# marsupialtail/quokka

Measured on AMD Instinct MI355X. Metric: rows/s, higher is better.
Workload: dtype f64; 1 GPU; TPC-H SF100 Q1, fused filter+group-by, 600037900 lineitem rows/GPU resident in HBM (BASELINE.json configs[1]); rows_per_gpu=600037900, query=Q1

## Files before the change

include/quokka_amd.h:

```cpp
#ifndef QUOKKA_AMD_H
#define QUOKKA_AMD_H

#include <stdint.h>

#ifdef __cplusplus
extern "C" {
#endif

int qk_init(int device);
int qk_device_count(int *out);
const char *qk_last_error(void);
const char *qk_build_arch(void);

int qk_dmalloc(uint64_t nbytes, void **dptr);
int qk_hmalloc_impl(uint64_t nbytes, void **hptr);
int qk_hfree(void *hptr);
int qk_dfree(void *dptr);
int qk_h2d(void *dst_dev, const void *src_host, uint64_t nbytes);
int qk_d2h(void *dst_host, const void *src_dev, uint64_t nbytes);
int qk_h2d_async(void *stream, void *dst_dev, const void *src_host,
                 uint64_t nbytes);
int qk_d2h_async(void *stream, void *dst_host, const void *src_dev,
                 uint64_t nbytes);
int qk_dmemset(void *dst_dev, int value, uint64_t nbytes);
int qk_fill_i64(void *stream, int64_t *dst_dev, int64_t value, uint64_t n);

int qk_stream_create(void **stream);
int qk_stream_destroy(void *stream);
int qk_stream_sync(void *stream);
int qk_event_create(void **ev);
int qk_event_destroy(void *ev);
int qk_event_record(void *ev, void *stream);
int qk_stream_wait_event(void *stream, void *ev);
int qk_timer_create(void **timer);
int qk_timer_destroy(void *timer);
int qk_timer_start(void *timer, void *stream);
int qk_timer_stop(void *timer, void *stream);
int qk_timer_elapsed_ms(void *timer, float *out_ms);

int qk_gen_lineitem(void *stream, uint64_t n, uint64_t row_offset, uint64_t seed,
                    int64_t n_parts, int64_t n_suppliers, int64_t n_orders,
                    int64_t *l_orderkey, int64_t *l_suppkey,
                    double *l_quantity, double *l_extendedprice,
                    double *l_discount, double *l_tax,
                    uint8_t *l_returnflag, uint8_t *l_linestatus,
                    int32_t *l_shipdate, int32_t *l_commitdate,
                    int32_t *l_receiptdate);

int qk_gen_orders(void *stream, uint64_t n, uint64_t row_offset, uint64_t seed,
                  int64_t n_customers, int64_t *o_orderkey, int64_t *o_custkey,
                  int32_t *o_orderdate, int32_t *o_shippriority,
                  uint8_t *o_orderpriority, double *o_totalprice,
                  int64_t li_n_parts);
int qk_gen_customer(void *stream, uint64_t n, uint64_t row_offset,
                    uint64_t seed, int64_t *c_custkey, uint8_t *c_mktsegment,
                    int32_t *c_nationkey);
int qk_gen_supplier(void *stream, uint64_t n, uint64_t row_offset,
                    uint64_t seed, int64_t *s_suppkey, int32_t *s_nationkey);
int qk_gen_aux(void *stream, uint64_t n, uint64_t row_offset, uint64_t seed,
               uint64_t salt, int mode, int64_t a, int64_t b,
               uint8_t *out_u8, double *out_f64);

int qk_q1_agg(void *stream, uint64_t n,
              const int32_t *l_shipdate, const double *l_quantity,
              const double *l_extendedprice, const double *l_discount,
              const double *l_tax, const uint8_t *l_returnflag,
              const uint8_t *l_linestatus, int32_t cutoff_date,
              double *out_dev );

int qk_q6_agg(void *stream, uint64_t n,
              const int32_t *l_shipdate, const double *l_quantity,
              const double *l_extendedprice, const double *l_discount,
              int32_t date_lo, int32_t date_hi,
              double disc_lo, double disc_hi, double qty_hi,
              double *out_dev );

int qk_filter_i32(void *stream, uint64_t n, const int32_t *col, int op,
                  int32_t value, uint32_t *out_idx, uint64_t *out_count_dev);
int qk_filter_u8(void *stream, uint64_t n, const uint8_t *col, int op,
                 uint8_t value, uint32_t *out_idx, uint64_t *out_count_dev);
int qk_filter_f64(void *stream, uint64_t n, const double *col, int op,
                  double value, uint32_t *out_idx, uint64_t *out_count_dev);

int qk_flag_gt_i32(void *stream, uint64_t n, const int32_t *a,
                   const int32_t *b, double *out);
int qk_mul_1md(void *stream, uint64_t n, const double *a, const double *b,
               double *out);

int qk_gather_i64(void *stream, uint64_t n_idx, const uint32_t *idx,
                  const int64_t *src, int64_t *dst);
int qk_gather_f64(void *stream, uint64_t n_idx, const uint32_t *idx,
                  const double *src, double *dst);
int qk_gather_i32(void *stream, uint64_t n_idx, const uint32_t *idx,
                  const int32_t *src, int32_t *dst);
int qk_gather_u8(void *stream, uint64_t n_idx, const uint32_t *idx,
                 const uint8_t *src, uint8_t *dst);

#define QK_JOIN_EMPTY INT64_MIN
int qk_join_build(void *stream, uint64_t n_build, const int64_t *keys,
                  uint32_t build_row_offset, int64_t *slot_keys,
                  int32_t *slot_head, int32_t *chain_next, uint64_t capacity);
int qk_join_probe(void *stream, uint64_t n_probe, const int64_t *keys,
                  const int64_t *slot_keys, const int32_t *slot_head,
                  const int32_t *chain_next, uint64_t capacity, int mode,
                  uint32_t *out_probe_idx, uint32_t *out_build_idx,
                  uint64_t out_capacity, uint64_t *out_cursor_dev);

int qk_build_u8eq(void *stream, uint64_t n, const int64_t *keys,
                  const uint8_t *flag, uint8_t flag_val, int64_t *slot_keys,
                  int32_t *slot_head, uint64_t capacity, uint32_t *bloom,
                  uint64_t bloom_mask);
int qk_q3_build_orders(void *stream, uint64_t n, const int64_t *o_orderkey,
                       const int64_t *o_custkey, const int32_t *o_orderdate,
                       int32_t date_lt, const int64_t *cust_keys,
                       const int32_t *cust_head, uint64_t cust_cap,
                       int64_t *slot_keys, int32_t *slot_head,
                       uint64_t capacity, uint32_t *bloom,
                       uint64_t bloom_mask, const uint32_t *cust_bloom,
                       uint64_t cust_bloom_mask);
int qk_q3_count_orders(void *stream, uint64_t n, const int64_t *o_custkey,
                       const int32_t *o_orderdate, int32_t date_lt,
                       const int64_t *cust_keys, const int32_t *cust_head,
                       uint64_t cust_cap, uint64_t *count_dev,
                       const uint32_t *cust_bloom, uint64_t cust_bloom_mask);
int qk_q3_probe_agg(void *stream, uint64_t n, const int64_t *l_orderkey,
                    const int32_t *l_shipdate, const double *l_price,
                    const double *l_disc, int32_t date_gt,
                    const int64_t *slot_keys, const int32_t *slot_head,
                    uint64_t capacity, double *slot_sums ,
                    uint64_t *match_count_dev );
int qk_q3_probe_agg_nt(void *stream, uint64_t n, const int64_t *l_orderkey,
                       const int32_t *l_shipdate, const double *l_price,
                       const double *l_disc, int32_t date_gt,
                       const int64_t *slot_keys, const int32_t *slot_head,
                       uint64_t capacity, double *slot_sums,
                       uint64_t *match_count_dev, const uint32_t *bloom,
                       uint64_t bloom_mask);
int qk_q3_probe_agg_nt4(void *stream, uint64_t n, const int64_t *l_orderkey,
                        const int32_t *l_shipdate, const double *l_price,
                        const double *l_disc, int32_t date_gt,
                        const int64_t *slot_keys, const int32_t *slot_head,
                        uint64_t capacity, double *slot_sums,
                        uint64_t *match_count_dev, const uint32_t *bloom,
                        uint64_t bloom_mask);
int qk_q3_extract(void *stream, const int64_t *slot_keys,
                  const int32_t *slot_head, const double *slot_sums,
                  uint64_t capacity, int64_t *out_keys, int32_t *out_row,
                  double *out_sums, uint64_t out_cap, uint64_t *cursor_dev);

int qk_build_keyval_i32(void *stream, uint64_t n, const int64_t *keys,
                        const int32_t *vals, uint32_t accept_mask,
                        int64_t *slot_keys, int32_t *slot_val,
                        uint64_t capacity, uint32_t *bloom,
                        uint64_t bloom_mask);
int qk_q5_build_orders(void *stream, uint64_t n, const int64_t *o_orderkey,
                       const int64_t *o_custkey, const int32_t *o_orderdate,
                       int32_t date_lo, int32_t date_hi,
                       const int64_t *cust_keys, const int32_t *cust_val,
                       uint64_t cust_cap, int64_t *slot_keys,
                       int32_t *slot_val, uint64_t capacity,
                       uint64_t *count_dev, uint32_t *bloom,
                       uint64_t bloom_mask, const uint32_t *cust_bloom,
                       uint64_t cust_bloom_mask);
int qk_q5_probe_agg(void *stream, uint64_t n, const int64_t *l_orderkey,
                    const int64_t *l_suppkey, const double *l_price,
                    const double *l_disc, const int64_t *ord_keys,
                    const int32_t *ord_val, uint64_t ord_cap,
                    const int64_t *supp_keys, const int32_t *supp_val,
                    uint64_t supp_cap, double *out25,
                    uint64_t *match_count_dev );

int qk_q5_probe_agg_nt(void *stream, uint64_t n, const int64_t *l_orderkey,
                       const int64_t *l_suppkey, const double *l_price,
                       const double *l_disc, const int64_t *ord_keys,
                       const int32_t *ord_val, uint64_t ord_cap,
                       const int64_t *supp_keys, const int32_t *supp_val,
                       uint64_t supp_cap, double *out25,
                       uint64_t *match_count_dev, const uint32_t *bloom,
                       uint64_t bloom_mask);

int qk_groupby_i64_sum(void *stream, uint64_t n, const int64_t *keys,
                       const void *vals_dev ,
                       const int32_t *agg_ops_dev ,
                       int nvals, int rstride ,
                       int64_t *table, uint64_t cap, uint64_t *n_inserted);
int qk_groupby_init(void *stream, int64_t *table, uint64_t cap, int rstride,
                    int nvals, const double *inits_dev);
int qk_fill_f64(void *stream, double *dst_dev, double value, uint64_t n);
int qk_groupby_extract(void *stream, const int64_t *table, int rstride,
                       int nvals, uint64_t cap, int64_t *out_keys,
                       double *out_sums ,
                       uint64_t out_cap, uint64_t *cursor);
int qk_groupby_extract_gt(void *stream, const int64_t *table, int rstride,
                          int nvals, uint64_t cap, int col, double threshold,
                          int64_t *out_keys, double *out_sums,
                          uint64_t out_cap, uint64_t *cursor);

int qk_partition_hist(void *stream, uint64_t n, const int64_t *keys,
                      uint32_t nparts, uint64_t *hist_dev);
int qk_partition_scatter(void *stream, uint64_t n, const int64_t *keys,
                         uint32_t nparts, uint64_t *cursors_dev,
                         uint32_t *out_idx);

int qk_sort_pairs_u64(void *stream, uint64_t n, uint64_t *keys,
                      uint32_t *payload, uint64_t *keys_tmp,
                      uint32_t *pay_tmp, int npasses);
int qk_map_f64_u64(void *stream, uint64_t n, const double *in, uint64_t *out);
int qk_map_i64_u64(void *stream, uint64_t n, const int64_t *in,
                   uint64_t *out);
int qk_iota_u32(void *stream, uint64_t n, uint32_t *out);
int qk_bnot_u64(void *stream, uint64_t n, uint64_t *x);

const char *qk_jit_last_error(void);
int qk_jit_filter_build(const char *c_expr, int ncols, const int *coltypes,
                        void **prog_out);
int qk_jit_filter_run(void *prog, void *stream, uint64_t n,
                      const void *const *col_ptrs, uint32_t *out_idx,
                      uint64_t *count_dev);
int qk_jit_map_build(const char *c_expr, int ncols, const int *coltypes,
                     void **prog_out);
int qk_jit_map_run(void *prog, void *stream, uint64_t n,
                   const void *const *col_ptrs, double *out_dev);
int qk_jit_agg_build(const char *pred_or_empty, const char *group_expr,
                     int ngroups, int naggs, const char *const *agg_exprs,
                     const int *agg_ops, int ncols, const int *coltypes,
                     void **prog_out);
int qk_jit_agg_run(void *prog, void *stream, uint64_t n,
                   const void *const *col_ptrs, double *out_dev);
int qk_jit_filter_free(void *prog);
uint64_t qk_jit_code_size(void *prog);

#define QK_UID_BYTES 128
int qk_comm_unique_id(uint8_t out[QK_UID_BYTES]);
int qk_comm_init(int rank, int world, const uint8_t uid[QK_UID_BYTES],
                 void **comm_out);
int qk_comm_destroy(void *comm);
int qk_alltoallv(void *stream, void *comm, int world, uint32_t elem_size,
                 const void *send_buf, const uint64_t *send_offsets,
                 const uint64_t *send_counts, void *recv_buf,
                 const uint64_t *recv_offsets, const uint64_t *recv_counts);
int qk_allreduce_f64(void *stream, void *comm, double *buf, uint64_t n);

int qk_pq_plain_copy(void *stream, uint64_t ntiles, const uint64_t *tiles,
                     const void *src_bytes, void *dst, uint32_t elem_size);
int qk_pq_rle_pages(void *stream, uint64_t npages, const uint64_t *ents,
                    const uint8_t *src_bytes, uint32_t *out);
int qk_str_dict_encode(void *stream, uint64_t n, const int64_t *offsets,
                       const uint8_t *bytes, uint64_t *slot_hash,
                       int32_t *slot_code, uint64_t capacity,
                       uint64_t *code_off, uint32_t *code_len,
                       uint8_t *arena, uint64_t *arena_cursor_dev,
                       uint32_t *counter_dev, uint32_t *out_codes);
int qk_str_dict_rehash(void *stream, uint32_t ncodes,
                       const uint64_t *code_off, const uint32_t *code_len,
                       const uint8_t *arena, uint64_t *slot_hash,
                       int32_t *slot_code, uint64_t capacity);
#define QK_LIKE_MAX_PAT 256
#define QK_LIKE_MAX_SEGS 16
typedef struct {
  uint32_t nseg;
  uint8_t anchor_start;
  uint8_t anchor_end;
  uint8_t exact;
  uint8_t pad_;
  uint16_t seg_off[QK_LIKE_MAX_SEGS];
  uint16_t seg_len[QK_LIKE_MAX_SEGS];
  uint32_t wild[QK_LIKE_MAX_PAT / 32];
  uint8_t pat[QK_LIKE_MAX_PAT];
} qk_like_pat;
int qk_like_compile(const uint8_t *pat, uint32_t len, int exact,
                    qk_like_pat *out);
int qk_str_like_i32(void *stream, uint64_t n, const int32_t *offsets,
                    const uint8_t *bytes, const qk_like_pat *pat, int negate,
                    uint8_t *out_flags);
int qk_str_like_i64(void *stream, uint64_t n, const int64_t *offsets,
                    const uint8_t *bytes, const qk_like_pat *pat, int negate,
                    uint8_t *out_flags);
int qk_str_like_path_i32(void *stream, uint64_t n, const int32_t *offsets,
                         const uint8_t *bytes, const qk_like_pat *pat,
                         int negate, int stage, uint8_t *out_flags);
int qk_str_like_path_i64(void *stream, uint64_t n, const int64_t *offsets,
                         const uint8_t *bytes, const qk_like_pat *pat,
                         int negate, int stage, uint8_t *out_flags);
int qk_str_like_host_i64(uint64_t n, const int64_t *offsets,
                         const uint8_t *bytes, const qk_like_pat *pat,
                         int negate, uint8_t *out_flags);
int qk_like_tile_bytes(void);
int qk_i64_combine(void *stream, uint64_t n, const int64_t *x,
                   const int64_t *y, int64_t scale, int64_t *out);
int qk_i64_shr(void *stream, uint64_t n, const int64_t *x, int shift,
               int64_t *out);
int qk_d2d(void *dst_dev, const void *src_dev, uint64_t nbytes);

int qk_snappy_pages(void *stream, uint64_t npages, const uint64_t *descs_dev,
                    const uint8_t *src_dev, uint8_t *dst_dev,
                    int64_t *out_dev);
int qk_gzip_pages(void *stream, uint64_t npages, const uint64_t *descs_dev,
                  const uint8_t *src_dev, uint8_t *dst_dev,
                  int64_t *out_dev);
#define QK_PQ_PAGE_FIELDS 10
int qk_pq_walk_pages(const uint8_t *buf, uint64_t start,
                     uint64_t total_len, int64_t num_values, int64_t *out,
                     int64_t max_pages, int64_t *n_out);

int qk_range_part_ids(void *stream, uint64_t n, const int64_t *keys,
                      int64_t per_range, uint32_t nparts, int64_t *out);

#define QK_CSV_MAX_DICT 32
int qk_csv_newlines(void *stream, uint64_t data_start, uint64_t n,
                    const uint8_t *bytes, uint64_t *out_pos,
                    uint64_t *out_count_dev);
int qk_csv_newlines_quoted(void *stream, uint64_t data_start, uint64_t n,
                           const uint8_t *bytes_dev, uint8_t quote_char,
                           uint64_t *out_pos_dev, uint64_t *out_count_dev);
int qk_csv_parse(void *stream, uint64_t nrows, const uint8_t *bytes,
                 uint64_t data_start, const uint64_t *nl_pos, uint8_t sep,
                 uint8_t quote_char , int ncols,
                 const int *coltypes, void *const *out_ptrs,
                 const uint64_t *dict_cands, const uint8_t *dict_lens,
                 const int *ncands, uint64_t *err_row);

#ifdef __cplusplus
}
#endif
#endif
```

quokka_amd/csrc/quokka_amd.hip:

```cpp

#include <hip/hip_runtime.h>
#include <stdint.h>
#include <stdio.h>
#include <string.h>
#include "../../include/quokka_amd.h"

#define WAVE 64

static __host__ __device__ inline uint64_t qk_min_u64(uint64_t a, uint64_t b) {
  return a < b ? a : b;
}
#define BLOCK 256
#define MAX_BLOCKS 2048

static __thread char g_err[512] = "";
static __thread int g_err_set = 0;

static int qk_fail(const char *where, hipError_t e) {
  snprintf(g_err, sizeof(g_err), "%s: %s", where, hipGetErrorString(e));
  g_err_set = 1;
  return (int)(e == hipSuccess ? hipErrorUnknown : e);
}
#define QK_TRY(where, expr)                                                    \
  do {                                                                         \
// ... 37 lines not shown
extern "C" int qk_d2h(void *dst, const void *src, uint64_t n) {
  QK_TRY("qk_d2h", hipMemcpy(dst, src, n, hipMemcpyDeviceToHost));
  return 0;
}
extern "C" int qk_h2d_async(void *stream, void *dst, const void *src,
                            uint64_t n) {
  QK_TRY("qk_h2d_async", hipMemcpyAsync(dst, src, n, hipMemcpyHostToDevice,
                                        (hipStream_t)stream));
  return 0;
}
extern "C" int qk_d2h_async(void *stream, void *dst, const void *src,
                            uint64_t n) {
  QK_TRY("qk_d2h_async", hipMemcpyAsync(dst, src, n, hipMemcpyDeviceToHost,
                                        (hipStream_t)stream));
  return 0;
}
extern "C" int qk_dmemset(void *dst, int value, uint64_t n) {
  QK_TRY("qk_dmemset", hipMemset(dst, value, n));
  return 0;
}

__global__ void k_fill_i64(int64_t *dst, int64_t v, uint64_t n) {
  uint64_t stride = (uint64_t)gridDim.x * blockDim.x;
  for (uint64_t i = (uint64_t)blockIdx.x * blockDim.x + threadIdx.x; i < n;
       i += stride)
    dst[i] = v;
}
extern "C" int qk_fill_i64(void *stream, int64_t *dst, int64_t v, uint64_t n) {
  if (!n) return 0;
  uint32_t blocks = (uint32_t)qk_min_u64(MAX_BLOCKS, (n + BLOCK - 1) / BLOCK);
  hipLaunchKernelGGL(k_fill_i64, dim3(blocks), dim3(BLOCK), 0,
                     (hipStream_t)stream, dst, v, n);
  QK_TRY("qk_fill_i64", hipGetLastError());
  return 0;
}

extern "C" int qk_stream_create(void **stream) {
  QK_TRY("qk_stream_create", hipStreamCreate((hipStream_t *)stream));
  return 0;
}
extern "C" int qk_stream_destroy(void *stream) {
  QK_TRY("qk_stream_destroy", hipStreamDestroy((hipStream_t)stream));
  return 0;
}
extern "C" int qk_stream_sync(void *stream) {
  QK_TRY("qk_stream_sync", hipStreamSynchronize((hipStream_t)stream));
  return 0;
}

extern "C" int qk_event_create(void **ev) {
  QK_TRY("qk_event_create",
         hipEventCreateWithFlags((hipEvent_t *)ev, hipEventDisableTiming));
  return 0;
}
extern "C" int qk_event_destroy(void *ev) {
  QK_TRY("qk_event_destroy", hipEventDestroy((hipEvent_t)ev));
  return 0;
}
extern "C" int qk_event_record(void *ev, void *stream) {
  QK_TRY("qk_event_record",
         hipEventRecord((hipEvent_t)ev, (hipStream_t)stream));
  return 0;
}
extern "C" int qk_stream_wait_event(void *stream, void *ev) {
  QK_TRY("qk_stream_wait_event",
         hipStreamWaitEvent((hipStream_t)stream, (hipEvent_t)ev, 0));
  return 0;
}

struct QkTimer {
  hipEvent_t start, stop;
};
extern "C" int qk_timer_create(void **timer) {
  QkTimer *t = new QkTimer();
  QK_TRY("qk_timer_create.start", hipEventCreate(&t->start));
  QK_TRY("qk_timer_create.stop", hipEventCreate(&t->stop));
  *timer = t;
  return 0;
}
extern "C" int qk_timer_destroy(void *timer) {
  QkTimer *t = (QkTimer *)timer;
  hipEventDestroy(t->start);
  hipEventDestroy(t->stop);
  delete t;
  return 0;
}
extern "C" int qk_timer_start(void *timer, void *stream) {
  QK_TRY("qk_timer_start",
         hipEventRecord(((QkTimer *)timer)->start, (hipStream_t)stream));
  return 0;
}
extern "C" int qk_timer_stop(void *timer, void *stream) {
  QK_TRY("qk_timer_stop",
         hipEventRecord(((QkTimer *)timer)->stop, (hipStream_t)stream));
  return 0;
}
extern "C" int qk_timer_elapsed_ms(void *timer, float *out_ms) {
  QkTimer *t = (QkTimer *)timer;
  QK_TRY("qk_timer_elapsed.sync", hipEventSynchronize(t->stop));
  QK_TRY("qk_timer_elapsed", hipEventElapsedTime(out_ms, t->start, t->stop));
  return 0;
}

__device__ __host__ inline uint64_t splitmix64(uint64_t x) {
  x += 0x9E3779B97F4A7C15ULL;
  x ^= x >> 30;
  x *= 0xBF58476D1CE4E5B9ULL;
  x ^= x >> 27;
  x *= 0x94D049BB133111EBULL;
  x ^= x >> 31;
  return x;
}

#define QK_ORDERDATE_LO 8035
#define QK_ORDERDATE_HI 10440
#define QK_RECEIPT_CUTOFF 9298

__global__ void k_gen_lineitem(uint64_t n, uint64_t row_offset, uint64_t seed,
                               int64_t n_parts, int64_t n_suppliers,
                               int64_t n_orders, int64_t *l_orderkey,
                               int64_t *l_suppkey, double *l_quantity,
                               double *l_extendedprice, double *l_discount,
                               double *l_tax, uint8_t *l_returnflag,
                               uint8_t *l_linestatus, int32_t *l_shipdate,
                               int32_t *l_commitdate,
                               int32_t *l_receiptdate) {
  uint64_t stride = (uint64_t)gridDim.x * blockDim.x;
  for (uint64_t i = (uint64_t)blockIdx.x * blockDim.x + threadIdx.x; i < n;
       i += stride) {
    uint64_t row = row_offset + i;
    uint64_t base = splitmix64(seed ^ 0x51A2B3C4D5E6F708ULL) ^
                    (row * 0x9E3779B97F4A7C15ULL);
    uint64_t h1 = splitmix64(base + 1),
             h2 = splitmix64(base + 2), h3 = splitmix64(base + 3),
             h4 = splitmix64(base + 4), h5 = splitmix64(base + 5),
             h6 = splitmix64(base + 6), h7 = splitmix64(base + 7),
             h8 = splitmix64(base + 8);
    uint64_t order_row = (row / 4) % (uint64_t)n_orders;
    uint64_t obase = splitmix64(seed ^ 0x0DE50DE50DE50DE5ULL) ^
                     (order_row * 0x9E3779B97F4A7C15ULL);
    int32_t odate = QK_ORDERDATE_LO +
        (int32_t)(splitmix64(obase + 1) %
                  (QK_ORDERDATE_HI - QK_ORDERDATE_LO + 1));
    int32_t ship = odate + 1 + (int32_t)(h1 % 121);
    int32_t receipt = ship + 1 + (int32_t)(h2 % 30);
    if (l_commitdate)
      l_commitdate[i] = odate + 30 + (int32_t)(splitmix64(base + 9) % 61);
    if (l_receiptdate) l_receiptdate[i] = receipt;
    if (l_shipdate) l_shipdate[i] = ship;
    if (l_returnflag)
      l_returnflag[i] =
          (receipt <= QK_RECEIPT_CUTOFF) ? ((h3 & 1) ? (uint8_t)0 : (uint8_t)2)
                                         : (uint8_t)1;
    if (l_linestatus) l_linestatus[i] = ship > QK_RECEIPT_CUTOFF ? 1 : 0;
    double qty = (double)(1 + (int32_t)(h4 % 50));
    if (l_quantity) l_quantity[i] = qty;
    if (l_extendedprice) {
      int64_t pk = 1 + (int64_t)(h5 % (uint64_t)n_parts);
      int64_t cents = 90000 + (pk / 10) % 20001 + 100 * (pk % 1000);
      l_extendedprice[i] = qty * ((double)cents / 100.0);
    }
    if (l_discount) l_discount[i] = (double)(h6 % 11) / 100.0;
    if (l_tax) l_tax[i] = (double)(h7 % 9) / 100.0;
    if (l_suppkey) l_suppkey[i] = 1 + (int64_t)(h8 % (uint64_t)n_suppliers);
    if (l_orderkey) {
      uint64_t orow = row / 4 % (uint64_t)n_orders;
      l_orderkey[i] = (int64_t)((orow / 8) * 32 + orow % 8) + 1;
    }
  }
}
extern "C" int qk_gen_lineitem(void *stream, uint64_t n, uint64_t row_offset,
                               uint64_t seed, int64_t n_parts,
                               int64_t n_suppliers, int64_t n_orders,
                               int64_t *l_orderkey, int64_t *l_suppkey,
                               double *l_quantity, double *l_extendedprice,
                               double *l_discount, double *l_tax,
                               uint8_t *l_returnflag, uint8_t *l_linestatus,
                               int32_t *l_shipdate, int32_t *l_commitdate,
                               int32_t *l_receiptdate) {
  if (!n) return 0;
  uint32_t blocks = (uint32_t)qk_min_u64(MAX_BLOCKS, (n + BLOCK - 1) / BLOCK);
  hipLaunchKernelGGL(k_gen_lineitem, dim3(blocks), dim3(BLOCK), 0,
                     (hipStream_t)stream, n, row_offset, seed, n_parts,
                     n_suppliers, n_orders, l_orderkey, l_suppkey, l_quantity,
                     l_extendedprice, l_discount, l_tax, l_returnflag,
                     l_linestatus, l_shipdate, l_commitdate, l_receiptdate);
  QK_TRY("qk_gen_lineitem", hipGetLastError());
  return 0;
}

__global__ void k_gen_orders(uint64_t n, uint64_t row_offset, uint64_t seed,
                             int64_t n_customers, int64_t *o_orderkey,
                             int64_t *o_custkey, int32_t *o_orderdate,
                             int32_t *o_shippriority,
                             uint8_t *o_orderpriority, double *o_totalprice,
                             int64_t li_n_parts) {
  uint64_t stride = (uint64_t)gridDim.x * blockDim.x;
  for (uint64_t i = (uint64_t)blockIdx.x * blockDim.x + threadIdx.x; i < n;
       i += stride) {
    uint64_t row = row_offset + i;
    uint64_t base = splitmix64(seed ^ 0x0DE50DE50DE50DE5ULL) ^
                    (row * 0x9E3779B97F4A7C15ULL);
    uint64_t h0 = splitmix64(base + 0), h1 = splitmix64(base + 1);
    if (o_orderkey) o_orderkey[i] = (int64_t)((row / 8) * 32 + row % 8) + 1;
    if (o_custkey) {
      int64_t ck = 1 + (int64_t)(h0 % (uint64_t)n_customers);
      if (ck % 3 == 0) ck -= 1;
      o_custkey[i] = ck;
    }
    if (o_orderdate)
      o_orderdate[i] = QK_ORDERDATE_LO +
          (int32_t)(h1 % (QK_ORDERDATE_HI - QK_ORDERDATE_LO + 1));
    if (o_shippriority) o_shippriority[i] = 0;
    if (o_orderpriority)
      o_orderpriority[i] = (uint8_t)(splitmix64(base + 2) % 5);
    if (o_totalprice) {
      double tp = 0.0;
      for (int j = 0; j < 4; j++) {
        uint64_t lrow = 4 * row + (uint64_t)j;
        uint64_t lbase = splitmix64(seed ^ 0x51A2B3C4D5E6F708ULL) ^
                         (lrow * 0x9E3779B97F4A7C15ULL);
        uint64_t h4 = splitmix64(lbase + 4), h5 = splitmix64(lbase + 5),
                 h6 = splitmix64(lbase + 6), h7 = splitmix64(lbase + 7);
        double qty = (double)(1 + (int32_t)(h4 % 50));
        int64_t pk = 1 + (int64_t)(h5 % (uint64_t)li_n_parts);
        int64_t cents = 90000 + (pk / 10) % 20001 + 100 * (pk % 1000);
        double price = qty * ((double)cents / 100.0);
        double disc = (double)(h6 % 11) / 100.0;
        double tax = (double)(h7 % 9) / 100.0;
        tp += price * (1.0 + tax) * (1.0 - disc);
      }
      o_totalprice[i] = tp;
    }
  }
}
extern "C" int qk_gen_orders(void *stream, uint64_t n, uint64_t row_offset,
                             uint64_t seed, int64_t n_customers,
                             int64_t *o_orderkey, int64_t *o_custkey,
                             int32_t *o_orderdate, int32_t *o_shippriority,
                             uint8_t *o_orderpriority, double *o_totalprice,
                             int64_t li_n_parts) {
  if (!n) return 0;
  uint32_t blocks = (uint32_t)qk_min_u64(MAX_BLOCKS, (n + BLOCK - 1) / BLOCK);
  hipLaunchKernelGGL(k_gen_orders, dim3(blocks), dim3(BLOCK), 0,
                     (hipStream_t)stream, n, row_offset, seed, n_customers,
                     o_orderkey, o_custkey, o_orderdate, o_shippriority,
                     o_orderpriority, o_totalprice, li_n_parts);
  QK_TRY("qk_gen_orders", hipGetLastError());
  return 0;
}

__global__ void k_gen_customer(uint64_t n, uint64_t row_offset, uint64_t seed,
                               int64_t *c_custkey, uint8_t *c_mktsegment,
                               int32_t *c_nationkey) {
  uint64_t stride = (uint64_t)gridDim.x * blockDim.x;
  for (uint64_t i = (uint64_t)blockIdx.x * blockDim.x + threadIdx.x; i < n;
       i += stride) {
    uint64_t row = row_offset + i;
    uint64_t h = splitmix64((seed ^ 0xC0573C0573C0573CULL) +
                            row * 0x9E3779B97F4A7C15ULL);
    if (c_custkey) c_custkey[i] = (int64_t)row + 1;
    if (c_mktsegment) c_mktsegment[i] = (uint8_t)(h % 5);
    if (c_nationkey) c_nationkey[i] = (int32_t)((h >> 32) % 25);
  }
}
extern "C" int qk_gen_customer(void *stream, uint64_t n, uint64_t row_offset,
                               uint64_t seed, int64_t *c_custkey,
                               uint8_t *c_mktsegment, int32_t *c_nationkey) {
  if (!n) return 0;
  uint32_t blocks = (uint32_t)qk_min_u64(MAX_BLOCKS, (n + BLOCK - 1) / BLOCK);
  hipLaunchKernelGGL(k_gen_customer, dim3(blocks), dim3(BLOCK), 0,
                     (hipStream_t)stream, n, row_offset, seed, c_custkey,
                     c_mktsegment, c_nationkey);
  QK_TRY("qk_gen_customer", hipGetLastError());
  return 0;
}


#define Q1_ACC_DECL(g)                                                         \
  double a##g##0 = 0, a##g##1 = 0, a##g##2 = 0, a##g##3 = 0, a##g##4 = 0,      \
         a##g##5 = 0;
#define Q1_ACC_ADD(g)                                                          \
  if (gid == g) {                                                              \
    a##g##0 += qty;                                                            \
    a##g##1 += price;                                                          \
    a##g##2 += disc_price;                                                     \
    a##g##3 += charge;                                                         \
    a##g##4 += disc;                                                           \
    a##g##5 += 1.0;                                                            \
  }
#define Q1_ACC_ROW()                                                           \
  do {                                                                         \
    double disc_price = price * (1.0 - disc);                                  \
    double charge = disc_price * (1.0 + tax);                                  \
    Q1_ACC_ADD(0) else Q1_ACC_ADD(1) else Q1_ACC_ADD(2) else Q1_ACC_ADD(       \
        3) else Q1_ACC_ADD(4) else Q1_ACC_ADD(5)                               \
  } while (0)

__device__ inline double wave_reduce(double v) {
  for (int off = WAVE / 2; off > 0; off >>= 1) v += __shfl_down(v, off);
  return v;
}

__global__ void __launch_bounds__(BLOCK) k_q1_agg(
    uint64_t n, const int32_t *__restrict__ shipdate,
    const double *__restrict__ quantity, const double *__restrict__ extprice,
    const double *__restrict__ discount, const double *__restrict__ tax_,
    const uint8_t *__restrict__ rflag, const uint8_t *__restrict__ lstat,
    int32_t cutoff, double *__restrict__ out) {
  Q1_ACC_DECL(0) Q1_ACC_DECL(1) Q1_ACC_DECL(2)
  Q1_ACC_DECL(3) Q1_ACC_DECL(4) Q1_ACC_DECL(5)

  uint64_t npairs = n / 2;
  uint64_t stride = (uint64_t)gridDim.x * blockDim.x;
  for (uint64_t p = (uint64_t)blockIdx.x * blockDim.x + threadIdx.x; p < npairs;
       p += stride) {
    uint64_t r = 2 * p;
    typedef double v2d __attribute__((ext_vector_type(2)));
    typedef int v2i __attribute__((ext_vector_type(2)));
    v2d q2 = __builtin_nontemporal_load(
        reinterpret_cast<const v2d *>(quantity + r));
    v2d p2 = __builtin_nontemporal_load(
        reinterpret_cast<const v2d *>(extprice + r));
    v2d d2 = __builtin_nontemporal_load(
        reinterpret_cast<const v2d *>(discount + r));
    v2d t2 = __builtin_nontemporal_load(
        reinterpret_cast<const v2d *>(tax_ + r));
    v2i s2 = __builtin_nontemporal_load(
        reinterpret_cast<const v2i *>(shipdate + r));
    uint8_t f0 = __builtin_nontemporal_load(&rflag[r]);
    uint8_t f1 = __builtin_nontemporal_load(&rflag[r + 1]);
    uint8_t l0 = __builtin_nontemporal_load(&lstat[r]);
    uint8_t l1 = __builtin_nontemporal_load(&lstat[r + 1]);
    if (s2.x <= cutoff) {
      int gid = (int)f0 * 2 + (int)l0;
      double qty = q2.x, price = p2.x, disc = d2.x, tax = t2.x;
      Q1_ACC_ROW();
    }
    if (s2.y <= cutoff) {
      int gid = (int)f1 * 2 + (int)l1;
      double qty = q2.y, price = p2.y, disc = d2.y, tax = t2.y;
      Q1_ACC_ROW();
    }
  }
  if (blockIdx.x == 0 && threadIdx.x == 0 && (n & 1)) {
    uint64_t r = n - 1;
    if (shipdate[r] <= cutoff) {
      int gid = (int)rflag[r] * 2 + (int)lstat[r];
      double qty = quantity[r], price = extprice[r], disc = discount[r],
             tax = tax_[r];
      Q1_ACC_ROW();
    }
  }

  __shared__ double lds[BLOCK / WAVE][36];
  int lane = threadIdx.x & (WAVE - 1);
  int wid = threadIdx.x / WAVE;
#define Q1_RED(g, j, var)                                                      \
  {                                                                            \
    double s = wave_reduce(var);                                               \
    if (lane == 0) lds[wid][g * 6 + j] = s;                                    \
  }
#define Q1_RED_G(g)                                                            \
  Q1_RED(g, 0, a##g##0) Q1_RED(g, 1, a##g##1) Q1_RED(g, 2, a##g##2)            \
  Q1_RED(g, 3, a##g##3) Q1_RED(g, 4, a##g##4) Q1_RED(g, 5, a##g##5)
  Q1_RED_G(0) Q1_RED_G(1) Q1_RED_G(2) Q1_RED_G(3) Q1_RED_G(4) Q1_RED_G(5)
  __syncthreads();
  if (threadIdx.x < 36) {
    double s = 0;
    for (int w = 0; w < BLOCK / WAVE; w++) s += lds[w][threadIdx.x];
    int g = threadIdx.x / 6, j = threadIdx.x % 6;
    if (s != 0.0) atomicAdd(&out[g * 8 + j], s);
  }
}

extern "C" int qk_q1_agg(void *stream, uint64_t n, const int32_t *shipdate,
                         const double *quantity, const double *extprice,
                         const double *discount, const double *tax,
                         const uint8_t *rflag, const uint8_t *lstat,
                         int32_t cutoff, double *out) {
  uint64_t npairs = n / 2;
  uint32_t blocks =
      (uint32_t)qk_min_u64(MAX_BLOCKS, (npairs + BLOCK - 1) / BLOCK);
  if (!blocks) blocks = 1;
  hipLaunchKernelGGL(k_q1_agg, dim3(blocks), dim3(BLOCK), 0,
                     (hipStream_t)stream, n, shipdate, quantity, extprice,
                     discount, tax, rflag, lstat, cutoff, out);
  QK_TRY("qk_q1_agg", hipGetLastError());
  return 0;
}

__global__ void __launch_bounds__(BLOCK) k_q6_agg(
    uint64_t n, const int32_t *__restrict__ shipdate,
    const double *__restrict__ quantity, const double *__restrict__ extprice,
    const double *__restrict__ discount, int32_t date_lo, int32_t date_hi,
    double disc_lo, double disc_hi, double qty_hi, double *__restrict__ out) {
  double rev = 0, cnt = 0;
  uint64_t npairs = n / 2;
  uint64_t stride = (uint64_t)gridDim.x * blockDim.x;
  for (uint64_t p = (uint64_t)blockIdx.x * blockDim.x + threadIdx.x; p < npairs;
       p += stride) {
    uint64_t r = 2 * p;
    typedef double v2d __attribute__((ext_vector_type(2)));
    typedef int v2i __attribute__((ext_vector_type(2)));
    v2d q2 = __builtin_nontemporal_load(
        reinterpret_cast<const v2d *>(quantity + r));
    v2d p2 = __builtin_nontemporal_load(
        reinterpret_cast<const v2d *>(extprice + r));
    v2d d2 = __builtin_nontemporal_load(
        reinterpret_cast<const v2d *>(discount + r));
    v2i s2 = __builtin_nontemporal_load(
        reinterpret_cast<const v2i *>(shipdate + r));
    if (s2.x >= date_lo && s2.x < date_hi && d2.x >= disc_lo &&
        d2.x <= disc_hi && q2.x < qty_hi) {
      rev += p2.x * d2.x;
      cnt += 1.0;
    }
    if (s2.y >= date_lo && s2.y < date_hi && d2.y >= disc_lo &&
        d2.y <= disc_hi && q2.y < qty_hi) {
      rev += p2.y * d2.y;
      cnt += 1.0;
    }
  }
  if (blockIdx.x == 0 && threadIdx.x == 0 && (n & 1)) {
    uint64_t r = n - 1;
    if (shipdate[r] >= date_lo && shipdate[r] < date_hi &&
        discount[r] >= disc_lo && discount[r] <= disc_hi &&
        quantity[r] < qty_hi) {
      rev += extprice[r] * discount[r];
      cnt += 1.0;
    }
  }
  __shared__ double lds[2][BLOCK / WAVE];
  int lane = threadIdx.x & (WAVE - 1);
  int wid = threadIdx.x / WAVE;
  double s0 = wave_reduce(rev), s1 = wave_reduce(cnt);
  if (lane == 0) {
    lds[0][wid] = s0;
    lds[1][wid] = s1;
  }
  __syncthreads();
  if (threadIdx.x < 2) {
    double s = 0;
    for (int w = 0; w < BLOCK / WAVE; w++) s += lds[threadIdx.x][w];
    if (s != 0.0) atomicAdd(&out[threadIdx.x], s);
  }
}
extern "C" int qk_q6_agg(void *stream, uint64_t n, const int32_t *shipdate,
                         const double *quantity, const double *extprice,
                         const double *discount, int32_t date_lo,
                         int32_t date_hi, double disc_lo, double disc_hi,
                         double qty_hi, double *out) {
  uint64_t npairs = n / 2;
  uint32_t blocks =
      (uint32_t)qk_min_u64(MAX_BLOCKS, (npairs + BLOCK - 1) / BLOCK);
  if (!blocks) blocks = 1;
  hipLaunchKernelGGL(k_q6_agg, dim3(blocks), dim3(BLOCK), 0,
                     (hipStream_t)stream, n, shipdate, quantity, extprice,
                     discount, date_lo, date_hi, disc_lo, disc_hi, qty_hi, out);
  QK_TRY("qk_q6_agg", hipGetLastError());
  return 0;
}


template <typename T>
__device__ inline bool cmp_op(T v, int op, T ref) {
  switch (op) {
  case 0: return v < ref;
  case 1: return v <= ref;
  case 2: return v > ref;
  case 3: return v >= ref;
  case 4: return v == ref;
  default: return v != ref;
  }
}

template <typename T>
__global__ void __launch_bounds__(BLOCK) k_filter_count(
    uint64_t n, const T *__restrict__ col, int op, T ref, uint64_t chunk,
    uint64_t *__restrict__ block_counts) {
  uint64_t lo = (uint64_t)blockIdx.x * chunk;
  uint64_t hi = qk_min_u64(n, lo + chunk);
  uint32_t cnt = 0;
  for (uint64_t r = lo + threadIdx.x; r < hi; r += BLOCK)
    cnt += cmp_op(col[r], op, ref) ? 1u : 0u;
  __shared__ uint32_t lds[BLOCK / WAVE];
  for (int off = WAVE / 2; off > 0; off >>= 1) cnt += __shfl_down(cnt, off);
  int lane = threadIdx.x & (WAVE - 1), wid = threadIdx.x / WAVE;
  if (lane == 0) lds[wid] = cnt;
  __syncthreads();
  if (threadIdx.x == 0) {
    uint64_t s = 0;
    for (int w = 0; w < BLOCK / WAVE; w++) s += lds[w];
    block_counts[blockIdx.x] = s;
  }
}

__global__ void k_scan_blocks(uint64_t nblocks, uint64_t *__restrict__ counts,
                              uint64_t *__restrict__ total) {
  if (blockIdx.x == 0 && threadIdx.x == 0) {
    uint64_t acc = 0;
    for (uint64_t b = 0; b < nblocks; b++) {
      uint64_t c = counts[b];
      counts[b] = acc;
      acc += c;
    }
    *total = acc;
  }
}

template <typename T>
__global__ void __launch_bounds__(BLOCK) k_filter_scatter(
    uint64_t n, const T *__restrict__ col, int op, T ref, uint64_t chunk,
    const uint64_t *__restrict__ block_offsets, uint32_t *__restrict__ out_idx) {
  uint64_t lo = (uint64_t)blockIdx.x * chunk;
  uint64_t hi = qk_min_u64(n, lo + chunk);
  __shared__ uint64_t base;
  __shared__ uint32_t wave_tot[BLOCK / WAVE];
  if (threadIdx.x == 0) base = block_offsets[blockIdx.x];
  __syncthreads();
  int lane = threadIdx.x & (WAVE - 1), wid = threadIdx.x / WAVE;
  for (uint64_t r0 = lo; r0 < hi; r0 += BLOCK) {
    uint64_t r = r0 + threadIdx.x;
    bool pass = r < hi && cmp_op(col[r], op, ref);
    uint64_t mask = __ballot(pass);
    uint32_t rank = __popcll(mask & ((1ULL << lane) - 1));
    uint32_t wtot = __popcll(mask);
    if (lane == 0) wave_tot[wid] = wtot;
    __syncthreads();
    uint32_t wbase = 0;
    for (int w = 0; w < wid; w++) wbase += wave_tot[w];
    if (pass) out_idx[base + wbase + rank] = (uint32_t)r;
    uint32_t btot = 0;
    for (int w = 0; w < BLOCK / WAVE; w++) btot += wave_tot[w];
    __syncthreads();
    if (threadIdx.x == 0) base += btot;
    __syncthreads();
  }
}

template <typename T>
static int qk_filter_impl(const char *who, void *stream, uint64_t n,
                          const T *col, int op, T value, uint32_t *out_idx,
                          uint64_t *out_count_dev) {
  if (!n) return 0;
  uint64_t rows_per_block = (n + MAX_BLOCKS - 1) / MAX_BLOCKS;
  rows_per_block = ((rows_per_block + BLOCK - 1) / BLOCK) * BLOCK;
  uint32_t blocks = (uint32_t)((n + rows_per_block - 1) / rows_per_block);
  static __thread uint64_t *scratch = nullptr;
  static __thread uint64_t scratch_cap = 0;
  if (scratch_cap < blocks) {
    if (scratch) hipFree(scratch);
    QK_TRY(who, hipMalloc(&scratch, (MAX_BLOCKS + 1) * sizeof(uint64_t)));
    scratch_cap = MAX_BLOCKS + 1;
  }
  hipLaunchKernelGGL(k_filter_count<T>, dim3(blocks), dim3(BLOCK), 0,
                     (hipStream_t)stream, n, col, op, value, rows_per_block,
                     scratch);
  hipLaunchKernelGGL(k_scan_blocks, dim3(1), dim3(1), 0, (hipStream_t)stream,
                     (uint64_t)blocks, scratch, out_count_dev);
  hipLaunchKernelGGL(k_filter_scatter<T>, dim3(blocks), dim3(BLOCK), 0,
                     (hipStream_t)stream, n, col, op, value, rows_per_block,
                     scratch, out_idx);
  QK_TRY(who, hipGetLastError());
  return 0;
}
extern "C" int qk_filter_i32(void *stream, uint64_t n, const int32_t *col,
                             int op, int32_t value, uint32_t *out_idx,
                             uint64_t *out_count_dev) {
  return qk_filter_impl("qk_filter_i32", stream, n, col, op, value, out_idx,
                        out_count_dev);
}
extern "C" int qk_filter_u8(void *stream, uint64_t n, const uint8_t *col,
                            int op, uint8_t value, uint32_t *out_idx,
                            uint64_t *out_count_dev) {
  return qk_filter_impl("qk_filter_u8", stream, n, col, op, value, out_idx,
                        out_count_dev);
}
extern "C" int qk_filter_f64(void *stream, uint64_t n, const double *col,
                             int op, double value, uint32_t *out_idx,
                             uint64_t *out_count_dev) {
  return qk_filter_impl("qk_filter_f64", stream, n, col, op, value, out_idx,
                        out_count_dev);
}

__global__ void k_flag_gt_i32(uint64_t n, const int32_t *__restrict__ a,
                              const int32_t *__restrict__ b,
                              double *__restrict__ out) {
  uint64_t stride = (uint64_t)gridDim.x * blockDim.x;
  for (uint64_t i = (uint64_t)blockIdx.x * blockDim.x + threadIdx.x; i < n;
       i += stride)
    out[i] = a[i] > b[i] ? 1.0 : 0.0;
}
extern "C" int qk_flag_gt_i32(void *stream, uint64_t n, const int32_t *a,
                              const int32_t *b, double *out) {
  if (!n) return 0;
  uint32_t blocks = (uint32_t)qk_min_u64(MAX_BLOCKS, (n + BLOCK - 1) / BLOCK);
  hipLaunchKernelGGL(k_flag_gt_i32, dim3(blocks), dim3(BLOCK), 0,
                     (hipStream_t)stream, n, a, b, out);
  QK_TRY("qk_flag_gt_i32", hipGetLastError());
  return 0;
}

__global__ void k_mul_1md(uint64_t n, const double *__restrict__ a,
                          const double *__restrict__ b,
                          double *__restrict__ out) {
  uint64_t stride = (uint64_t)gridDim.x * blockDim.x;
  for (uint64_t i = (uint64_t)blockIdx.x * blockDim.x + threadIdx.x; i < n;
       i += stride)
    out[i] = a[i] * (1.0 - b[i]);
}
extern "C" int qk_mul_1md(void *stream, uint64_t n, const double *a,
                          const double *b, double *out) {
  if (!n) return 0;
  uint32_t blocks = (uint32_t)qk_min_u64(MAX_BLOCKS, (n + BLOCK - 1) / BLOCK);
  hipLaunchKernelGGL(k_mul_1md, dim3(blocks), dim3(BLOCK), 0,
                     (hipStream_t)stream, n, a, b, out);
  QK_TRY("qk_mul_1md", hipGetLastError());
  return 0;
}

template <typename T>
__global__ void k_gather(uint64_t n, const uint32_t *__restrict__ idx,
                         const T *__restrict__ src, T *__restrict__ dst) {
  uint64_t stride = (uint64_t)gridDim.x * blockDim.x;
  for (uint64_t i = (uint64_t)blockIdx.x * blockDim.x + threadIdx.x; i < n;
       i += stride)
    dst[i] = src[idx[i]];
}
template <typename T>
static int qk_gather_impl(const char *who, void *stream, uint64_t n,
                          const uint32_t *idx, const T *src, T *dst) {
  if (!n) return 0;
  uint32_t blocks = (uint32_t)qk_min_u64(MAX_BLOCKS, (n + BLOCK - 1) / BLOCK);
  hipLaunchKernelGGL(k_gather<T>, dim3(blocks), dim3(BLOCK), 0,
                     (hipStream_t)stream, n, idx, src, dst);
  QK_TRY(who, hipGetLastError());
  return 0;
}
extern "C" int qk_gather_i64(void *s, uint64_t n, const uint32_t *i,
                             const int64_t *src, int64_t *dst) {
  return qk_gather_impl("qk_gather_i64", s, n, i, src, dst);
}
extern "C" int qk_gather_f64(void *s, uint64_t n, const uint32_t *i,
                             const double *src, double *dst) {
  return qk_gather_impl("qk_gather_f64", s, n, i, src, dst);
}
extern "C" int qk_gather_i32(void *s, uint64_t n, const uint32_t *i,
                             const int32_t *src, int32_t *dst) {
  return qk_gather_impl("qk_gather_i32", s, n, i, src, dst);
}
extern "C" int qk_gather_u8(void *s, uint64_t n, const uint32_t *i,
                            const uint8_t *src, uint8_t *dst) {
  return qk_gather_impl("qk_gather_u8", s, n, i, src, dst);
}


__device__ inline uint64_t slot_of(int64_t key, uint64_t cap) {
  return splitmix64((uint64_t)key) & (cap - 1);
}

__device__ inline uint32_t bloom_word_mask(int64_t key, uint64_t bloom_mask,
                                           uint64_t *word_idx) {
  uint64_t h = splitmix64((uint64_t)key ^ 0xB10011B10011B100ULL);
  *word_idx = (h & bloom_mask) >> 5;
  uint32_t b1 = (uint32_t)(h >> 40) & 31u, b2 = (uint32_t)(h >> 48) & 31u;
  return (1u << b1) | (1u << b2);
}
__device__ inline void bloom_set(uint32_t *bloom, uint64_t bloom_mask,
                                 int64_t key) {
  uint64_t w;
  uint32_t m = bloom_word_mask(key, bloom_mask, &w);
  atomicOr(&bloom[w], m);
}
__device__ inline bool bloom_test(const uint32_t *bloom, uint64_t bloom_mask,
                                  int64_t key) {
  uint64_t w;
  uint32_t m = bloom_word_mask(key, bloom_mask, &w);
  return (bloom[w] & m) == m;
}

__global__ void __launch_bounds__(BLOCK) k_join_build2(
    uint64_t n, const int64_t *__restrict__ keys, uint32_t row_offset,
    int64_t *__restrict__ slot_keys, int32_t *__restrict__ slot_head,
    int32_t *__restrict__ chain_next, uint64_t cap) {
  uint64_t stride = (uint64_t)gridDim.x * blockDim.x;
// ... 3029 lines not shown
```

Before: 154.8 billion rows/s.

## Use contiguous per-block tile ranges with occupancy-sized grid for Q1 aggregation

Replaces the grid-stride Q1 kernel with one that splits the input into 512-row tiles and gives each block a contiguous run of them. The grid is sized to the number of blocks that can be resident at once, taken from an occupancy query and cached per device. Flags are read as 16-bit pairs and group counts are kept as integers. The old row-pair kernel remains as a fallback when the column pointers are misaligned. The aim is better streaming locality and fewer, fully resident blocks, at the cost of per-block tail imbalance and extra host-side queries on first call.

```diff
diff --git a/include/quokka_amd.h b/include/quokka_amd.h
--- a/include/quokka_amd.h
+++ b/include/quokka_amd.h
@@ -67,6 +67,8 @@
               const double *l_tax, const uint8_t *l_returnflag,
               const uint8_t *l_linestatus, int32_t cutoff_date,
               double *out_dev );
+int qk_q1_tile_rows(void);
+int qk_q1_grid_blocks(int *out);
 
 int qk_q6_agg(void *stream, uint64_t n,
               const int32_t *l_shipdate, const double *l_quantity,
diff --git a/quokka_amd/csrc/quokka_amd.hip b/quokka_amd/csrc/quokka_amd.hip
--- a/quokka_amd/csrc/quokka_amd.hip
+++ b/quokka_amd/csrc/quokka_amd.hip
@@ -363,7 +363,7 @@
   return v;
 }
 
-__global__ void __launch_bounds__(BLOCK) k_q1_agg(
+__global__ void __launch_bounds__(BLOCK) k_q1_agg_rowpair(
     uint64_t n, const int32_t *__restrict__ shipdate,
     const double *__restrict__ quantity, const double *__restrict__ extprice,
     const double *__restrict__ discount, const double *__restrict__ tax_,
@@ -435,14 +435,172 @@
   }
 }
 
+#define Q1_TILE (2 * BLOCK)
+
+typedef double q1_v2d __attribute__((ext_vector_type(2)));
+typedef int q1_v2i __attribute__((ext_vector_type(2)));
+struct Q1Tile {
+  q1_v2d q, p, d, t;
+  q1_v2i s;
+  uint16_t f, l;
+};
+
+#define Q1S_LOAD(T_, r0, lo)                                                   \
+  do {                                                                         \
+    T_.q = __builtin_nontemporal_load(                                         \
+        reinterpret_cast<const q1_v2d *>((quantity + (r0)) + (lo)));           \
+    T_.p = __builtin_nontemporal_load(                                         \
+        reinterpret_cast<const q1_v2d *>((extprice + (r0)) + (lo)));           \
+    T_.d = __builtin_nontemporal_load(                                         \
+        reinterpret_cast<const q1_v2d *>((discount + (r0)) + (lo)));           \
+    T_.t = __builtin_nontemporal_load(                                         \
+        reinterpret_cast<const q1_v2d *>((tax_ + (r0)) + (lo)));               \
+    T_.s = __builtin_nontemporal_load(                                         \
+        reinterpret_cast<const q1_v2i *>((shipdate + (r0)) + (lo)));           \
+    T_.f = __builtin_nontemporal_load(                                         \
+        reinterpret_cast<const uint16_t *>((rflag + (r0)) + (lo)));            \
+    T_.l = __builtin_nontemporal_load(                                         \
+        reinterpret_cast<const uint16_t *>((lstat + (r0)) + (lo)));            \
+  } while (0)
+
+#define Q1S_ACC_DECL(g)                                                        \
+  double b##g##0 = 0, b##g##1 = 0, b##g##2 = 0, b##g##3 = 0, b##g##4 = 0;      \
+  uint32_t n##g = 0;
+#define Q1S_ACC_ADD(g)                                                         \
+  if (gid == g) {                                                              \
+    b##g##0 += qty;                                                            \
+    b##g##1 += price;                                                          \
+    b##g##2 += disc_price;                                                     \
+    b##g##3 += charge;                                                         \
+    b##g##4 += disc;                                                           \
+    n##g += 1;                                                                 \
+  }
+#define Q1S_ACC_ROW()                                                          \
+  do {                                                                         \
+    double disc_price = price * (1.0 - disc);                                  \
+    double charge = disc_price * (1.0 + tax);                                  \
+    Q1S_ACC_ADD(0) else Q1S_ACC_ADD(1) else Q1S_ACC_ADD(2) else Q1S_ACC_ADD(   \
+        3) else Q1S_ACC_ADD(4) else Q1S_ACC_ADD(5)                             \
+  } while (0)
+#define Q1S_ACC_TILE(T_)                                                       \
+  do {                                                                         \
+    if (T_.s.x <= cutoff) {                                                    \
+      int gid = (int)(T_.f & 0xff) * 2 + (int)(T_.l & 0xff);                   \
+      double qty = T_.q.x, price = T_.p.x, disc = T_.d.x, tax = T_.t.x;        \
+      Q1S_ACC_ROW();                                                           \
+    }                                                                          \
+    if (T_.s.y <= cutoff) {                                                    \
+      int gid = (int)(T_.f >> 8) * 2 + (int)(T_.l >> 8);                       \
+      double qty = T_.q.y, price = T_.p.y, disc = T_.d.y, tax = T_.t.y;        \
+      Q1S_ACC_ROW();                                                           \
+    }                                                                          \
+  } while (0)
+
+__global__ void __launch_bounds__(BLOCK) k_q1_agg(
+    uint64_t n, const int32_t *__restrict__ shipdate,
+    const double *__restrict__ quantity, const double *__restrict__ extprice,
+    const double *__restrict__ discount, const double *__restrict__ tax_,
+    const uint8_t *__restrict__ rflag, const uint8_t *__restrict__ lstat,
+    int32_t cutoff, double *__restrict__ out) {
+  Q1S_ACC_DECL(0) Q1S_ACC_DECL(1) Q1S_ACC_DECL(2)
+  Q1S_ACC_DECL(3) Q1S_ACC_DECL(4) Q1S_ACC_DECL(5)
+
+  const uint64_t ntiles = n / Q1_TILE;
+  const uint32_t lo = 2 * threadIdx.x;
+  const uint64_t per = ntiles / gridDim.x, rem = ntiles % gridDim.x;
+  const uint64_t first = blockIdx.x * per + qk_min_u64(blockIdx.x, rem);
+  const uint64_t cnt = per + (blockIdx.x < rem ? 1 : 0);
+  uint64_t r0 = first * Q1_TILE;
+  for (uint64_t i = 0; i < cnt; i++, r0 += Q1_TILE) {
+    Q1Tile a;
+    Q1S_LOAD(a, r0, lo);
+    __builtin_amdgcn_sched_barrier(0);
+    Q1S_ACC_TILE(a);
+  }
+  if (blockIdx.x == 0) {
+    for (uint64_t r = ntiles * Q1_TILE + threadIdx.x; r < n; r += BLOCK) {
+      if (shipdate[r] <= cutoff) {
+        int gid = (int)rflag[r] * 2 + (int)lstat[r];
+        double qty = quantity[r], price = extprice[r], disc = discount[r],
+               tax = tax_[r];
+        Q1S_ACC_ROW();
+      }
+    }
+  }
+
+  __shared__ double lds[BLOCK / WAVE][36];
+  int lane = threadIdx.x & (WAVE - 1);
+  int wid = threadIdx.x / WAVE;
+#define Q1S_RED(g, j, var)                                                     \
+  {                                                                            \
+    double s = wave_reduce(var);                                               \
+    if (lane == 0) lds[wid][g * 6 + j] = s;                                    \
+  }
+#define Q1S_RED_G(g)                                                           \
+  Q1S_RED(g, 0, b##g##0) Q1S_RED(g, 1, b##g##1) Q1S_RED(g, 2, b##g##2)         \
+  Q1S_RED(g, 3, b##g##3) Q1S_RED(g, 4, b##g##4) Q1S_RED(g, 5, (double)n##g)
+  Q1S_RED_G(0) Q1S_RED_G(1) Q1S_RED_G(2) Q1S_RED_G(3) Q1S_RED_G(4) Q1S_RED_G(5)
+  __syncthreads();
+  if (threadIdx.x < 36) {
+    double s = 0;
+    for (int w = 0; w < BLOCK / WAVE; w++) s += lds[w][threadIdx.x];
+    int g = threadIdx.x / 6, j = threadIdx.x % 6;
+    if (s != 0.0) atomicAdd(&out[g * 8 + j], s);
+  }
+}
+
+static int q1_resident_blocks(int *out) {
+  static int cache[64];
+  int dev = 0;
+  QK_TRY("qk_q1_agg.device", hipGetDevice(&dev));
+  if (dev < 0 || dev >= 64 || !cache[dev]) {
+    int per_cu = 0, cus = 0;
+    QK_TRY("qk_q1_agg.occupancy",
+           hipOccupancyMaxActiveBlocksPerMultiprocessor(
+               &per_cu, k_q1_agg, BLOCK, 0));
+    QK_TRY("qk_q1_agg.cus",
+           hipDeviceGetAttribute(&cus, hipDeviceAttributeMultiprocessorCount,
+                                 dev));
+    int v = per_cu * cus;
+    if (v <= 0) v = MAX_BLOCKS;
+    if (dev < 0 || dev >= 64) {
+      *out = v;
+      return 0;
+    }
+    cache[dev] = v;
+  }
+  *out = cache[dev];
+  return 0;
+}
+
+extern "C" int qk_q1_tile_rows(void) { return Q1_TILE; }
+extern "C" int qk_q1_grid_blocks(int *out) { return q1_resident_blocks(out); }
+
 extern "C" int qk_q1_agg(void *stream, uint64_t n, const int32_t *shipdate,
                          const double *quantity, const double *extprice,
                          const double *discount, const double *tax,
                          const uint8_t *rflag, const uint8_t *lstat,
                          int32_t cutoff, double *out) {
-  uint64_t npairs = n / 2;
-  uint32_t blocks =
-      (uint32_t)qk_min_u64(MAX_BLOCKS, (npairs + BLOCK - 1) / BLOCK);
+  uintptr_t mis = (((uintptr_t)quantity | (uintptr_t)extprice |
+                    (uintptr_t)discount | (uintptr_t)tax) & 15) |
+                  ((uintptr_t)shipdate & 7) |
+                  (((uintptr_t)rflag | (uintptr_t)lstat) & 1);
+  if (mis) {
+    uint64_t npairs = n / 2;
+    uint32_t blocks =
+        (uint32_t)qk_min_u64(MAX_BLOCKS, (npairs + BLOCK - 1) / BLOCK);
+    if (!blocks) blocks = 1;
+    hipLaunchKernelGGL(k_q1_agg_rowpair, dim3(blocks), dim3(BLOCK), 0,
+                       (hipStream_t)stream, n, shipdate, quantity, extprice,
+                       discount, tax, rflag, lstat, cutoff, out);
+    QK_TRY("qk_q1_agg", hipGetLastError());
+    return 0;
+  }
+  int resident = 0;
+  int rc = q1_resident_blocks(&resident);
+  if (rc) return rc;
+  uint64_t ntiles = n / Q1_TILE;
+  uint32_t blocks = (uint32_t)qk_min_u64((uint64_t)resident, ntiles);
   if (!blocks) blocks = 1;
   hipLaunchKernelGGL(k_q1_agg, dim3(blocks), dim3(BLOCK), 0,
                      (hipStream_t)stream, n, shipdate, quantity, extprice,
```

New measurement: 166.5 billion rows/s, median of 6. 7.6% higher.
